# dawn-search/dawnsearch

Measured on AMD Instinct MI355X. Metric: queries/sec, exact cosine top-k over a 384-d f32 index resident in HBM, higher is better.
Workload: dtype f32 (exact scores; int8 MFMA upper-bound filter over 5-bit / int8 shadows)

## Files before the change

### dawnsearch_amd/csrc/scan_f6.hip

```cpp
#include <type_traits>

#include "kernels.hpp"
#include "rotate384.hpp"
#include "wave_topk.hpp"

namespace dawn {

typedef int i32x8_t __attribute__((ext_vector_type(8)));
typedef uint32_t u32x2 __attribute__((ext_vector_type(2)));

constexpr uint32_t F6_KS_DW = 384;
constexpr uint32_t F6_TILE_DW = 3 * F6_KS_DW;
constexpr float F6_MAX = 7.5f;

__device__ __forceinline__ uint32_t f6_encode_mag(float t, float* deq) {
    t = fminf(t, F6_MAX);
    const int e = t < 1.0f ? 0 : t < 2.0f ? 1 : t < 4.0f ? 2 : 3;
    const float step = e <= 1 ? 0.125f : e == 2 ? 0.25f : 0.5f;
    float qn = rintf(t / step);
    if (e == 3) qn = fminf(qn, 15.0f);
    *deq = qn * step;
    const int q = (int)qn;
    return e == 0 ? (uint32_t)q : (uint32_t)((e << 3) + (q - 8));
}
__device__ __forceinline__ uint32_t f6_encode(float v, float inv_s, float* deq) {
    float d;
    const uint32_t c = f6_encode_mag(fabsf(v) * inv_s, &d);
    *deq = v < 0.f ? -d : d;
    return c | (v < 0.f ? 32u : 0u);
}

template <int RT>
__device__ __forceinline__ void rows_to_f6s_pair(const void* __restrict__ xv, uint32_t* __restrict__ out, float2* __restrict__ meta,
                                                 const uint32_t pair, uint32_t n_valid) {
    constexpr int NC = 6;
    __shared__ float sh[4];
    __shared__ float sh_e[4][NC];
    const int tid = threadIdx.x, lane = tid & 63, wave = tid >> 6;
    const uint32_t r = tid >> 3, part = tid & 7;
    const uint32_t row = pair * 32u + r;
    f32x4 v[12];
#pragma unroll
    for (int j = 0; j < 12; ++j) {
        v[j] = f32x4{0.f, 0.f, 0.f, 0.f};
        if (row < n_valid) {
            const uint32_t c4 = part + 8 * j;
            if (RT == 0) {
                v[j] = reinterpret_cast<const f32x4*>(xv)[(size_t)row * ROW_F4 + c4];
            } else {
                const u32x4 w = reinterpret_cast<const u32x4*>(xv)[frag_chunk(row, (int)(c4 >> 1))];
                const uint32_t w0 = (c4 & 1u) ? w.z : w.x, w1 = (c4 & 1u) ? w.w : w.y;
                v[j] = f32x4{bf16_lo(w0), bf16_hi(w0), bf16_lo(w1), bf16_hi(w1)};
            }
        }
    }
    rotate384_rowpart(v, part, lane);
    float amax = 0.f;
#pragma unroll
    for (int j = 0; j < 12; ++j)
        amax = fmaxf(amax, fmaxf(fmaxf(fabsf(v[j].x), fabsf(v[j].y)), fmaxf(fabsf(v[j].z), fabsf(v[j].w))));
#pragma unroll
    for (int o = 32; o >= 1; o >>= 1) amax = fmaxf(amax, __shfl_xor(amax, o));
    if (lane == 0) sh[wave] = amax;
    __syncthreads();
    const int w0 = wave & ~1;
    amax = fmaxf(sh[w0], sh[w0 + 1]);
    const float s0 = fmaxf(amax, 1e-20f) / F6_MAX;
    float e2c[NC];
#pragma unroll
    for (int ci = 0; ci < NC; ++ci) {
        const float inv_s = 1.0f / (s0 * (1.0f - 0.08f * ci)), s = s0 * (1.0f - 0.08f * ci);
        float e2 = 0.f;
#pragma unroll
        for (int j = 0; j < 12; ++j) {
            const float vv[4] = {v[j].x, v[j].y, v[j].z, v[j].w};
#pragma unroll
            for (int i = 0; i < 4; ++i) {
                float dq;
                (void)f6_encode(vv[i], inv_s, &dq);
                const float dx = vv[i] - s * dq;
                e2 = __builtin_fmaf(dx, dx, e2);
            }
        }
        e2 += __shfl_xor(e2, 1);
        e2 += __shfl_xor(e2, 2);
        e2 += __shfl_xor(e2, 4);
#pragma unroll
        for (int o2 = 32; o2 >= 8; o2 >>= 1) e2 = fmaxf(e2, __shfl_xor(e2, o2));
        e2c[ci] = e2;
    }
    if (lane == 0) {
#pragma unroll
        for (int ci = 0; ci < NC; ++ci) sh_e[wave][ci] = e2c[ci];
    }
    __syncthreads();
    float best_e2 = 0.f, s = s0;
#pragma unroll
    for (int ci = 0; ci < NC; ++ci) {
        const float m = fmaxf(sh_e[w0][ci], sh_e[w0 + 1][ci]);
        if (ci == 0 || m < best_e2) {
            best_e2 = m;
            s = s0 * (1.0f - 0.08f * ci);
        }
    }
    const float inv_s = 1.0f / s;
    const uint32_t tile = pair * 2u + (r >> 4), r16 = r & 15u;
    uint32_t* o = out + (size_t)tile * F6_TILE_DW;
    const int base = lane & ~7;
#pragma unroll
    for (int j = 0; j < 12; ++j) {
        const float vv[4] = {v[j].x, v[j].y, v[j].z, v[j].w};
        uint32_t c24 = 0;
#pragma unroll
        for (int i = 0; i < 4; ++i) {
            float dq;
            c24 |= f6_encode(vv[i], inv_s, &dq) << (6 * i);
        }
        const uint32_t c0 = __shfl(c24, base + 0), c1 = __shfl(c24, base + 1), c2 = __shfl(c24, base + 2), c3 = __shfl(c24, base + 3);
        const uint32_t c4 = __shfl(c24, base + 4), c5 = __shfl(c24, base + 5), c6 = __shfl(c24, base + 6), c7 = __shfl(c24, base + 7);
        uint32_t d = 0;
        switch (part) {
            case 0: d = c0 | (c1 << 24); break;
            case 1: d = (c1 >> 8) | (c2 << 16); break;
            case 2: d = (c2 >> 16) | (c3 << 8); break;
            case 3: d = c4 | (c5 << 24); break;
            case 4: d = (c5 >> 8) | (c6 << 16); break;
            case 5: d = (c6 >> 16) | (c7 << 8); break;
            default: break;
        }
        const uint32_t ks = (uint32_t)j >> 2, kb = (uint32_t)j & 3u, l = kb * 16u + r16;
        if (part < 4u) o[ks * F6_KS_DW + l * 4u + part] = d;
        else if (part < 6u) o[ks * F6_KS_DW + 256u + l * 2u + (part - 4u)] = d;
    }
    if ((tid & 127) == 0) {
        meta[tile] = float2{inv_s, sqrtf(best_e2) * 1.0101f * 1.001f + 1e-9f};
    }
}

template <int RT>
__global__ __launch_bounds__(256) void rows_to_f6s_kernel(const void* __restrict__ xv, uint32_t* __restrict__ out,
                                                           float2* __restrict__ meta, uint32_t first_pair, uint32_t n_valid) {
    rows_to_f6s_pair<RT>(xv, out, meta, first_pair + blockIdx.x, n_valid);
}

template <int RT>
__global__ __launch_bounds__(256) void rows_to_f6s_list_kernel(const void* __restrict__ xv, uint32_t* __restrict__ out,
                                                                float2* __restrict__ meta, const uint32_t* __restrict__ list,
                                                                const uint32_t* __restrict__ count, uint32_t end_pair, uint32_t n_valid) {
    if (blockIdx.x >= *count) return;
    const uint32_t pair = list[blockIdx.x];
    if (pair >= end_pair) return;
    rows_to_f6s_pair<RT>(xv, out, meta, pair, n_valid);
}

void launch_rows_to_f6s(const void* d_rows, int rt, void* d_shadow, void* d_meta, size_t first_row, size_t n_valid, hipStream_t stream) {
    const uint32_t first_pair = (uint32_t)(first_row / 32);
    const uint32_t end_pair = (uint32_t)((n_valid + 31) / 32);
    if (end_pair <= first_pair) return;
    if (rt == ROW_BF16)
        hipLaunchKernelGGL(rows_to_f6s_kernel<1>, dim3(end_pair - first_pair), dim3(256), 0, stream, d_rows,
                           reinterpret_cast<uint32_t*>(d_shadow), reinterpret_cast<float2*>(d_meta), first_pair, (uint32_t)n_valid);
    else
        hipLaunchKernelGGL(rows_to_f6s_kernel<0>, dim3(end_pair - first_pair), dim3(256), 0, stream, d_rows,
                           reinterpret_cast<uint32_t*>(d_shadow), reinterpret_cast<float2*>(d_meta), first_pair, (uint32_t)n_valid);
}

void launch_rows_to_f6s_list(const void* d_rows, int rt, void* d_shadow, void* d_meta, const uint32_t* d_list, const uint32_t* d_count,
                             uint32_t max_list, size_t prefix_rows, size_t n_valid, hipStream_t stream) {
    const uint32_t end_pair = (uint32_t)((prefix_rows + 31) / 32);
    if (max_list == 0 || end_pair == 0) return;
    if (rt == ROW_BF16)
        hipLaunchKernelGGL(rows_to_f6s_list_kernel<1>, dim3(max_list), dim3(256), 0, stream, d_rows, reinterpret_cast<uint32_t*>(d_shadow),
                           reinterpret_cast<float2*>(d_meta), d_list, d_count, end_pair, (uint32_t)n_valid);
    else
        hipLaunchKernelGGL(rows_to_f6s_list_kernel<0>, dim3(max_list), dim3(256), 0, stream, d_rows, reinterpret_cast<uint32_t*>(d_shadow),
                           reinterpret_cast<float2*>(d_meta), d_list, d_count, end_pair, (uint32_t)n_valid);
}

__global__ __launch_bounds__(64) void prep_queries_f6_kernel(const float* __restrict__ q, int n_q, uint32_t* __restrict__ qf6,
                                                              float2* __restrict__ qmeta) {
    __shared__ unsigned char codes[EM];
    const int b = blockIdx.x, lane = threadIdx.x;
    float v[6];
#pragma unroll
    for (int j = 0; j < 6; ++j) v[j] = b < n_q ? q[(size_t)b * EM + lane + 64 * j] : 0.f;
    rotate384_wave(v, lane);
    float amax = 0.f;
#pragma unroll
    for (int j = 0; j < 6; ++j) amax = fmaxf(amax, fabsf(v[j]));
#pragma unroll
    for (int o = 32; o >= 1; o >>= 1) amax = fmaxf(amax, __shfl_xor(amax, o));
    const float sq = fmaxf(amax, 1e-20f) / F6_MAX, inv = 1.0f / sq;
    float e2 = 0.f;
#pragma unroll
    for (int j = 0; j < 6; ++j) {
        float dq;
        const uint32_t c = f6_encode(v[j], inv, &dq);
        codes[lane + 64 * j] = b < n_q ? (unsigned char)c : (unsigned char)0;
        const float dx = v[j] - sq * dq;
        e2 = __builtin_fmaf(dx, dx, e2);
    }
#pragma unroll
    for (int o = 32; o >= 1; o >>= 1) e2 += __shfl_xor(e2, o);
    __syncthreads();
    const int g = b >> 4, c16 = b & 15;
    for (int w = lane; w < 72; w += 64) {
        const int kbk = w / 6, d = w % 6;
        uint32_t word = 0;
        const int first = (32 * d) / 6, last = (32 * d + 31) / 6;
        for (int i = first; i <= last && i < 32; ++i) {
            const int sh = 6 * i - 32 * d;
            const uint32_t c = codes[32 * kbk + i];
            word |= sh >= 0 ? (c << sh) : (c >> (-sh));
        }
        const int ks = kbk >> 2, kb = kbk & 3;
        qf6[(((size_t)g * 3 + ks) * 64 + kb * 16 + c16) * 6 + d] = word;
    }
    if (lane == 0) qmeta[b] = float2{sq, b < n_q ? sqrtf(e2) * 1.001f + 1e-9f : 0.f};
}

void launch_prep_queries_f6(const float* d_q, int n_q, void* d_qf6, void* d_qmeta, hipStream_t stream) {
    hipLaunchKernelGGL(prep_queries_f6_kernel, dim3(BATCH_QT), dim3(64), 0, stream, d_q, n_q, reinterpret_cast<uint32_t*>(d_qf6),
                       reinterpret_cast<float2*>(d_qmeta));
}

__device__ __forceinline__ i32x8_t f6_load_a(const uint32_t* tile, int ks, int lane) {
    const u32x4 lo = *reinterpret_cast<const u32x4*>(tile + ks * F6_KS_DW + lane * 4);
    const u32x2 hi = *reinterpret_cast<const u32x2*>(tile + ks * F6_KS_DW + 256 + lane * 2);
    return i32x8_t{(int)lo.x, (int)lo.y, (int)lo.z, (int)lo.w, (int)hi.x, (int)hi.y, 0, 0};
}

__global__ __launch_bounds__(64) void f6_dense_scores_kernel(const uint32_t* __restrict__ x, const float2* __restrict__ meta,
                                                              uint32_t n_rows, const uint32_t* __restrict__ qf6,
                                                              const float2* __restrict__ qmeta, int n_q, float* __restrict__ out) {
    const int lane = threadIdx.x;
    const uint32_t tile = blockIdx.x;
    const uint32_t* t = x + (size_t)tile * F6_TILE_DW;
    const float2 mt = meta[tile];
    const float s = __builtin_amdgcn_rcpf(mt.x);
    i32x8_t a[3];
#pragma unroll
    for (int ks = 0; ks < 3; ++ks) a[ks] = f6_load_a(t, ks, lane);
    for (int g = 0; g * 16 < n_q; ++g) {
        f32x4 acc = {0.f, 0.f, 0.f, 0.f};
#pragma unroll
        for (int ks = 0; ks < 3; ++ks) {
            const uint32_t* bp = qf6 + (((size_t)g * 3 + ks) * 64 + lane) * 6;
            const i32x8_t bv = {(int)bp[0], (int)bp[1], (int)bp[2], (int)bp[3], (int)bp[4], (int)bp[5], 0, 0};
            acc = __builtin_amdgcn_mfma_scale_f32_16x16x128_f8f6f4(a[ks], bv, acc, 2, 2, 0, 0x7F7F7F7F, 0, 0x7F7F7F7F);
        }
        const int qi = 16 * g + (lane & 15);
        const float2 qm = qmeta[qi];
        const float k2 = (1.015f + mt.y) * qm.y;
#pragma unroll
        for (int r = 0; r < 4; ++r) {
            const uint32_t row = tile * 16u + 4u * (uint32_t)(lane >> 4) + (uint32_t)r;
            if (qi < n_q && row < n_rows && row < (uint32_t)BATCH_CAP)
                out[(size_t)qi * BATCH_CAP + row] = __builtin_fmaf(acc[r], s * qm.x, mt.y + k2);
        }
    }
}

void launch_f6_dense_scores(const void* d_f6, const void* d_meta, uint32_t n_rows, const float* d_q, int B, void* d_qf6, void* d_qmeta,
                            float* d_out, hipStream_t stream) {
    launch_prep_queries_f6(d_q, B, d_qf6, d_qmeta, stream);
    const uint32_t n = n_rows < (uint32_t)BATCH_CAP ? n_rows : (uint32_t)BATCH_CAP;
    const uint32_t tiles = (n + 15u) / 16u;
    if (tiles == 0) return;
    hipLaunchKernelGGL(f6_dense_scores_kernel, dim3(tiles), dim3(64), 0, stream, reinterpret_cast<const uint32_t*>(d_f6),
                       reinterpret_cast<const float2*>(d_meta), n_rows, reinterpret_cast<const uint32_t*>(d_qf6),
                       reinterpret_cast<const float2*>(d_qmeta), B, d_out);
}


constexpr int F6_RING = 3;
constexpr uint32_t F6_STAGE = 1344;

template <bool DENSE>
__global__ __launch_bounds__(256) void scan_f6_pass_kernel(const uint32_t* __restrict__ x, const float2* __restrict__ meta, uint32_t n_rows,
                                                            uint32_t stride, uint32_t n_visits, const uint32_t* __restrict__ qf6,
                                                            const float2* __restrict__ qmeta, int n_q, const float* __restrict__ tau,
                                                            uint32_t* __restrict__ cnt, uint2* __restrict__ cand, uint32_t seg_cap,
                                                            float* __restrict__ dense, uint32_t stagger, int mark_lost) {
    __shared__ uint32_t stage[4][F6_STAGE][3];
    const int lane = threadIdx.x & 63;
    const int wave = __builtin_amdgcn_readfirstlane(threadIdx.x >> 6);
    const uint32_t G = gridDim.x;
    const uint32_t n_mine = n_visits > blockIdx.x ? (n_visits - blockIdx.x + G - 1u) / G : 0u;
    const uint32_t p0 = n_mine ? ((uint32_t)wave * stagger) % n_mine : 0u;
    auto visit_of = [&](uint32_t pos) __attribute__((always_inline)) -> uint32_t {
        if (n_mine == 0u) return 0u;
        uint32_t q = p0 + pos;
        q = q >= n_mine ? q - n_mine : q;
        q = q >= n_mine ? q % n_mine : q;
        return blockIdx.x + q * G;
    };
    uint32_t vis = 0;
    u32x4 alo[F6_RING][3];
    u32x2 ahi[F6_RING][3];
#define DAWN_F6_LD4(DST, PTR, OFF) asm volatile("global_load_dwordx4 %0, %1, %2 offset:" #OFF : "=v"(DST) : "v"(off4), "s"(PTR))
#define DAWN_F6_LD2(DST, PTR, OFF) asm volatile("global_load_dwordx2 %0, %1, %2 offset:" #OFF : "=v"(DST) : "v"(off2), "s"(PTR))
    const uint32_t off4 = (uint32_t)lane * 16u, off2 = 1024u + (uint32_t)lane * 8u;
    auto load_tile = [&](int slot, uint32_t v) __attribute__((always_inline)) {
        const uint32_t* p4 = x + (size_t)(v < n_visits ? v * stride : 0u) * F6_TILE_DW;
        const uint32_t* p2 = p4;
        DAWN_F6_LD4(alo[slot][0], p4, 0);
        DAWN_F6_LD2(ahi[slot][0], p2, 0);
        DAWN_F6_LD4(alo[slot][1], p4, 1536);
        DAWN_F6_LD2(ahi[slot][1], p2, 1536);
        DAWN_F6_LD4(alo[slot][2], p4, 3072);
        DAWN_F6_LD2(ahi[slot][2], p2, 3072);
    };
    auto take = [&](int slot, int ks, auto n_tag) __attribute__((always_inline)) -> i32x8_t {
        constexpr int N = decltype(n_tag)::value;
        int o0, o1, o2, o3, o4, o5;
        if constexpr (N >= 0)
            asm volatile("s_waitcnt vmcnt(%12)\n\tv_mov_b32 %0, %6\n\tv_mov_b32 %1, %7\n\tv_mov_b32 %2, %8\n\tv_mov_b32 %3, %9\n\t"
                         "v_mov_b32 %4, %10\n\tv_mov_b32 %5, %11"
                         : "=&v"(o0), "=&v"(o1), "=&v"(o2), "=&v"(o3), "=&v"(o4), "=&v"(o5)
                         : "v"(alo[slot][ks].x), "v"(alo[slot][ks].y), "v"(alo[slot][ks].z), "v"(alo[slot][ks].w), "v"(ahi[slot][ks].x),
                           "v"(ahi[slot][ks].y), "n"(N));
        else
            asm volatile("v_mov_b32 %0, %6\n\tv_mov_b32 %1, %7\n\tv_mov_b32 %2, %8\n\tv_mov_b32 %3, %9\n\tv_mov_b32 %4, %10\n\t"
                         "v_mov_b32 %5, %11"
                         : "=&v"(o0), "=&v"(o1), "=&v"(o2), "=&v"(o3), "=&v"(o4), "=&v"(o5)
                         : "v"(alo[slot][ks].x), "v"(alo[slot][ks].y), "v"(alo[slot][ks].z), "v"(alo[slot][ks].w), "v"(ahi[slot][ks].x),
                           "v"(ahi[slot][ks].y));
        return i32x8_t{o0, o1, o2, o3, o4, o5, 0, 0};
    };
#pragma unroll
    for (int d = 0; d < F6_RING; ++d) load_tile(d, visit_of((uint32_t)d));
    i32x8_t bq[4][3];
    float thrA[4], thrB[4], thrC[4], sq_l[4], dqn_l[4], tau_l[4];
#pragma unroll
    for (int gg = 0; gg < 4; ++gg) {
        const int g = 4 * wave + gg;
        const int qi = 16 * g + (lane & 15);
#pragma unroll
        for (int ks = 0; ks < 3; ++ks) {
            const uint32_t* bp = qf6 + (((size_t)g * 3 + ks) * 64 + lane) * 6;
            const u32x2 b01 = *reinterpret_cast<const u32x2*>(bp), b23 = *reinterpret_cast<const u32x2*>(bp + 2),
                        b45 = *reinterpret_cast<const u32x2*>(bp + 4);
            bq[gg][ks] = i32x8_t{(int)b01.x, (int)b01.y, (int)b23.x, (int)b23.y, (int)b45.x, (int)b45.y, 0, 0};
        }
        const float2 qm = qmeta[qi];
        sq_l[gg] = qm.x;
        dqn_l[gg] = qm.y;
        tau_l[gg] = (!DENSE && qi < n_q) ? tau[qi] : POS_INF;
        thrA[gg] = 1.0f / qm.x;
        thrB[gg] = tau_l[gg] - 1.015f * qm.y;
        thrC[gg] = -(1.0f + qm.y);
    }
    uint32_t n_stage = 0;
    uint32_t(*st)[3] = stage[wave];
    const uint32_t seg = blockIdx.x % (uint32_t)BATCH_CAND_SEGS;
    auto flush = [&]() __attribute__((always_inline)) {
        asm volatile("s_waitcnt lgkmcnt(0)" ::: "memory");
        for (uint32_t i = lane; i < n_stage; i += 64u) {
            const uint32_t ub = st[i][0], row = st[i][1], qi = st[i][2];
            const uint32_t pos = atomicAdd(&cnt[(size_t)qi * BATCH_CAND_SEGS + seg], 1u);
            if (pos < seg_cap) cand[((size_t)qi * BATCH_CAND_SEGS + seg) * seg_cap + pos] = uint2{ub, row};
        }
        n_stage = 0;
    };

    bool lost = false;
    while (vis < n_mine) {
      for (int it = 0; it < 16 && vis < n_mine && (DENSE || n_stage <= F6_STAGE - 1024u); ++it, vis += (uint32_t)F6_RING) {
#pragma unroll
        for (int d = 0; d < F6_RING; ++d) {
            if (vis + (uint32_t)d >= n_mine) break;
            const uint32_t v = visit_of(vis + (uint32_t)d);
            const uint32_t tile = v * stride;
            const float2 mt = meta[tile];
            i32x8_t av[3];
            av[0] = take(d, 0, std::integral_constant<int, 6 * (F6_RING - 1)>());
            av[1] = take(d, 1, std::integral_constant<int, -1>());
            av[2] = take(d, 2, std::integral_constant<int, -1>());
            load_tile(d, visit_of(vis + (uint32_t)d + (uint32_t)F6_RING));
            f32x4 acc[4];
#pragma unroll
            for (int gg = 0; gg < 4; ++gg) {
                acc[gg] = f32x4{0.f, 0.f, 0.f, 0.f};
#pragma unroll
                for (int ks = 0; ks < 3; ++ks)
                    acc[gg] = __builtin_amdgcn_mfma_scale_f32_16x16x128_f8f6f4(av[ks], bq[gg][ks], acc[gg], 2, 2, 0, 0x7F7F7F7F, 0,
                                                                                0x7F7F7F7F);
            }
            const float s = __builtin_amdgcn_rcpf(mt.x);
            const uint32_t row0 = tile * 16u + 4u * (uint32_t)(lane >> 4);
            if constexpr (DENSE) {
#pragma unroll
                for (int gg = 0; gg < 4; ++gg) {
                    const int qi = 16 * (4 * wave + gg) + (lane & 15);
                    const float k2 = (1.015f + mt.y) * dqn_l[gg];
#pragma unroll
                    for (int r = 0; r < 4; ++r) {
                        const uint32_t si = v * 16u + 4u * (uint32_t)(lane >> 4) + (uint32_t)r;
                        if (qi < n_q && si < (uint32_t)BATCH_CAP)
                            dense[(size_t)qi * BATCH_CAP + si] =
                                row0 + (uint32_t)r < n_rows ? __builtin_fmaf(acc[gg][r], s * sq_l[gg], mt.y + k2) : NEG_INF;
                    }
                }
            } else {
                bool any = false;
                float thr[4];
#pragma unroll
                for (int gg = 0; gg < 4; ++gg) {
                    thr[gg] = __builtin_fmaf(__builtin_fmaf(mt.y, thrC[gg], thrB[gg]), mt.x * thrA[gg], -0.02f);
                    any = any || fmaxf(fmaxf(acc[gg][0], acc[gg][1]), fmaxf(acc[gg][2], acc[gg][3])) > thr[gg];
                }
                if (__any(any)) {
#pragma unroll
                    for (int gg = 0; gg < 4; ++gg) {
                        const uint32_t qi = (uint32_t)(16 * (4 * wave + gg) + (lane & 15));
                        const float g1 = s * sq_l[gg], g0 = mt.y + (1.015f + mt.y) * dqn_l[gg];
#pragma unroll
                        for (int r = 0; r < 4; ++r) {
                            const float ub = __builtin_fmaf(acc[gg][r], g1, g0);
                            const bool hit = acc[gg][r] > thr[gg] && ub > tau_l[gg] && row0 + (uint32_t)r < n_rows;
                            const unsigned long long m = __ballot(hit);
                            if (m) {
                                if (hit) {
                                    const uint32_t slot = n_stage + (uint32_t)__popcll(m & ((1ull << lane) - 1ull));
                                    if (slot < F6_STAGE) {
                                        st[slot][0] = __builtin_bit_cast(uint32_t, ub);
                                        st[slot][1] = row0 + (uint32_t)r;
                                        st[slot][2] = qi;
                                    } else {
                                        lost = true;
                                    }
                                }
                                n_stage += (uint32_t)__popcll(m);
                                if (n_stage > F6_STAGE) n_stage = F6_STAGE;
                            }
                        }
                    }
                }
            }
        }
      }
      if (!DENSE && n_stage > 0u) flush();
    }
    asm volatile("s_waitcnt vmcnt(0)" ::: "memory");
#undef DAWN_F6_LD4
#undef DAWN_F6_LD2
    if (!DENSE && mark_lost && __any(lost)) {
        const uint32_t qi = (uint32_t)(64 * wave + lane);
        if ((int)qi < n_q) atomicAdd(&cnt[(size_t)qi * BATCH_CAND_SEGS + seg], seg_cap + 1u);
    }
}

constexpr int F6L_GROUP = 8;
constexpr uint32_t F6L_GROUP_BYTES = F6L_GROUP * F6_TILE_DW * 4u;
constexpr uint32_t F6L_STAGE = 448;
constexpr uint32_t F6L_FLUSH_AT = 192;
struct F6PassLds {
    uint32_t tiles[2][F6L_GROUP_BYTES / 4];
    uint32_t stage[8][F6L_STAGE][3];
};

template <int MODE>
__global__ __launch_bounds__(512) void scan_f6_pass_lds_kernel(const uint32_t* __restrict__ x, const float2* __restrict__ meta,
                                                                uint32_t n_rows, uint32_t n_tiles, const uint32_t* __restrict__ qf6,
                                                                const float2* __restrict__ qmeta, int n_q, const float* __restrict__ tau,
                                                                uint32_t* __restrict__ cnt, uint2* __restrict__ cand, uint32_t seg_cap) {
    extern __shared__ __attribute__((aligned(16))) unsigned char f6l_raw[];
    F6PassLds& L = *reinterpret_cast<F6PassLds*>(f6l_raw);
    const int lane = threadIdx.x & 63;
    const int wave = __builtin_amdgcn_readfirstlane(threadIdx.x >> 6);
    const int qw = wave & 3, half = wave >> 2;
    const uint32_t G = gridDim.x;
    const uint32_t n_groups = (n_tiles + (uint32_t)F6L_GROUP - 1u) / (uint32_t)F6L_GROUP;
    i32x8_t bq[4][3];
    float thrP[4], thrQ[4], sq_l[4], dqn_l[4];
#pragma unroll
    for (int gg = 0; gg < 4; ++gg) {
        const int g = 4 * qw + gg;
        const int qi = 16 * g + (lane & 15);
#pragma unroll
        for (int ks = 0; ks < 3; ++ks) {
            const uint32_t* bp = qf6 + (((size_t)g * 3 + ks) * 64 + lane) * 6;
            const u32x2 b01 = *reinterpret_cast<const u32x2*>(bp), b23 = *reinterpret_cast<const u32x2*>(bp + 2),
                        b45 = *reinterpret_cast<const u32x2*>(bp + 4);
            bq[gg][ks] = i32x8_t{(int)b01.x, (int)b01.y, (int)b23.x, (int)b23.y, (int)b45.x, (int)b45.y, 0, 0};
        }
        const float2 qm = qmeta[qi];
        sq_l[gg] = qm.x;
        dqn_l[gg] = qm.y;
        const float tau_q = qi < n_q ? tau[qi] : POS_INF;
        thrP[gg] = (tau_q - 1.015f * qm.y) / qm.x;
        thrQ[gg] = -(1.0f + qm.y) / qm.x;
    }
    uint32_t n_stage = 0;
    uint32_t(*st)[3] = L.stage[wave];
    const uint32_t seg = blockIdx.x % (uint32_t)BATCH_CAND_SEGS;
    bool lost = false;

    const uint32_t lds0 = (uint32_t)(size_t)(__attribute__((address_space(3))) unsigned char*)f6l_raw;
    const uint32_t o4 = (uint32_t)threadIdx.x * 16u, o2 = 32768u + (uint32_t)threadIdx.x * 8u, om = (uint32_t)(lane & 7) * 8u;
    const uint32_t o4b = o4 + 8192u, o4c = o4 + 16384u, o4d = o4 + 24576u;
    u32x4 pa0, pa1, pa2, pa3, pb0, pb1, pb2, pb3;
    u32x2 pa4, pb4, pam, pbm;
#define DAWN_F6L_PREFETCH(P0, P1, P2, P3, P4, PM, GRP)                                                                         \
    do {                                                                                                                      \
        const uint32_t g_ = (GRP) < n_groups ? (GRP) : n_groups - 1u;         \
        const unsigned char* xb_ = reinterpret_cast<const unsigned char*>(x) + (size_t)g_ * F6L_GROUP_BYTES;                  \
        const float2* mb_ = meta + (size_t)g_ * F6L_GROUP;                                                                    \
        asm volatile("global_load_dwordx4 %0, %6, %11 nt\n\tglobal_load_dwordx4 %1, %7, %11 nt\n\t"                           \
                     "global_load_dwordx4 %2, %8, %11 nt\n\tglobal_load_dwordx4 %3, %9, %11 nt\n\t"                           \
                     "global_load_dwordx2 %4, %10, %11 nt\n\tglobal_load_dwordx2 %5, %12, %13"                                \
                     : "=&v"(P0), "=&v"(P1), "=&v"(P2), "=&v"(P3), "=&v"(P4), "=&v"(PM)                                       \
                     : "v"(o4), "v"(o4b), "v"(o4c), "v"(o4d), "v"(o2), "s"(xb_), "v"(om), "s"(mb_)                            \
                     : "memory");                                                                                             \
    } while (0)
#define DAWN_F6L_LAND(P0, P1, P2, P3, P4, PM, BUF, MX, MY)                                                                     \
    do {                                                                                                                      \
        const uint32_t a4_ = lds0 + (BUF) + o4, a2_ = lds0 + (BUF) + (uint32_t)threadIdx.x * 8u;                              \
        asm volatile("s_waitcnt vmcnt(6)\n\tds_write_b128 %2, %4\n\tds_write_b128 %2, %5 offset:8192\n\t"                    \
                     "ds_write_b128 %2, %6 offset:16384\n\tds_write_b128 %2, %7 offset:24576\n\t"                            \
                     "ds_write_b64 %3, %8 offset:32768\n\tv_mov_b32 %0, %9\n\tv_mov_b32 %1, %10"                             \
                     : "=&v"(MX), "=&v"(MY)                                                                                   \
                     : "v"(a4_), "v"(a2_), "v"(P0), "v"(P1), "v"(P2), "v"(P3), "v"(P4), "v"(PM.x), "v"(PM.y)                  \
                     : "memory");                                                                                             \
    } while (0)
#define DAWN_F6L_BARRIER() asm volatile("s_waitcnt lgkmcnt(0)\n\ts_barrier" ::: "memory")

    auto compute = [&](const unsigned char* tb, uint32_t grp, int cmx, int cmy, auto mid) __attribute__((always_inline)) {
        auto read_tile = [&](int t, i32x8_t (&av)[3]) __attribute__((always_inline)) {
#pragma unroll
            for (int ks = 0; ks < 3; ++ks) {
                const unsigned char* f = tb + (uint32_t)t * (F6_TILE_DW * 4u) + (uint32_t)ks * (F6_KS_DW * 4u);
                const u32x4 lo = *reinterpret_cast<const u32x4*>(f + lane * 16);
                const u32x2 hi = *reinterpret_cast<const u32x2*>(f + 1024 + lane * 8);
                av[ks] = i32x8_t{(int)lo.x, (int)lo.y, (int)lo.z, (int)lo.w, (int)hi.x, (int)hi.y, 0, 0};
            }
        };
        constexpr int NT = F6L_GROUP / 2;
        i32x8_t av[2][3];
        f32x4 acc[2][4];
        read_tile(half, av[0]);
#pragma unroll
        for (int k = 0; k <= NT; ++k) {
            if (k + 1 < NT) read_tile(half + 2 * (k + 1), av[(k + 1) & 1]);
            if (k < NT) {
#pragma unroll
                for (int gg = 0; gg < 4; ++gg) acc[k & 1][gg] = f32x4{0.f, 0.f, 0.f, 0.f};
#pragma unroll
                for (int ks = 0; ks < 3; ++ks)
#pragma unroll
                    for (int gg = 0; gg < 4; ++gg)
                        acc[k & 1][gg] = __builtin_amdgcn_mfma_scale_f32_16x16x128_f8f6f4(av[k & 1][ks], bq[gg][ks], acc[k & 1][gg], 2, 2, 0,
                                                                                           0x7F7F7F7F, 0, 0x7F7F7F7F);
            }
            if (k >= 1) {
                const int t = half + 2 * (k - 1);
                const f32x4(&ac)[4] = acc[(k - 1) & 1];
                const uint32_t tile = grp * (uint32_t)F6L_GROUP + (uint32_t)t;
                const float2 mt = float2{__builtin_bit_cast(float, __builtin_amdgcn_readlane(cmx, t)),
                                         __builtin_bit_cast(float, __builtin_amdgcn_readlane(cmy, t))};
                const float sx = mt.x, sxy = mt.x * mt.y;
                unsigned long long mk[4][4], any_m = 0ull;
                float thr[4];
#pragma unroll
                for (int gg = 0; gg < 4; ++gg) {
                    thr[gg] = __builtin_fmaf(sx, thrP[gg], __builtin_fmaf(sxy, thrQ[gg], -0.02f));
#pragma unroll
                    for (int r = 0; r < 4; ++r) {
                        mk[gg][r] = __ballot(ac[gg][r] > thr[gg]);
                        any_m |= mk[gg][r];
                    }
                }
                if (MODE != 1 && any_m != 0ull) {
                    const float s = __builtin_amdgcn_rcpf(mt.x);
                    const uint32_t row0 = tile * 16u + 4u * (uint32_t)(lane >> 4);
#pragma unroll
                    for (int gg = 0; gg < 4; ++gg) {
                        if ((mk[gg][0] | mk[gg][1] | mk[gg][2] | mk[gg][3]) == 0ull) continue;
                        const uint32_t qi = (uint32_t)(16 * (4 * qw + gg) + (lane & 15));
                        const float g1 = s * sq_l[gg], g0 = mt.y + (1.015f + mt.y) * dqn_l[gg];
#pragma unroll
                        for (int r = 0; r < 4; ++r) {
                            if (mk[gg][r] == 0ull) continue;
                            const bool hit = ac[gg][r] > thr[gg] && row0 + (uint32_t)r < n_rows;
                            const unsigned long long m = __ballot(hit);
                            if (hit) {
                                const uint32_t slot = n_stage + (uint32_t)__popcll(m & ((1ull << lane) - 1ull));
                                if (slot < F6L_STAGE) {
                                    st[slot][0] = __builtin_bit_cast(uint32_t, __builtin_fmaf(ac[gg][r], g1, g0));
                                    st[slot][1] = row0 + (uint32_t)r;
                                    st[slot][2] = qi;
                                } else {
                                    lost = true;
                                }
                            }
                            n_stage += (uint32_t)__popcll(m);
                            if (n_stage > F6L_STAGE) n_stage = F6L_STAGE;
                        }
                    }
                }
                if constexpr (MODE == 1) {
                    const float sum = (ac[0][0] + ac[1][1]) + (ac[2][2] + ac[3][3]);
                    if (sum == 1.2345e30f) lost = true;
                }
            }
            if (k == 1) mid();
        }
    };
    auto flush = [&]() __attribute__((always_inline)) {
        for (uint32_t i = lane; i < n_stage; i += 64u) {
            const uint32_t ub = st[i][0], row = st[i][1], qi = st[i][2];
            const uint32_t pos = atomicAdd(&cnt[(size_t)qi * BATCH_CAND_SEGS + seg], 1u);
            if (pos < seg_cap) cand[((size_t)qi * BATCH_CAND_SEGS + seg) * seg_cap + pos] = uint2{ub, row};
        }
        n_stage = 0;
        asm volatile("s_waitcnt vmcnt(0)" ::: "memory");
    };

    uint32_t grp = blockIdx.x;
    if (grp < n_groups) {
        const unsigned char* tb0 = reinterpret_cast<const unsigned char*>(L.tiles[0]);
        const unsigned char* tb1 = reinterpret_cast<const unsigned char*>(L.tiles[1]);
        int mx0, my0, mx1, my1;
        DAWN_F6L_PREFETCH(pa0, pa1, pa2, pa3, pa4, pam, grp);
        DAWN_F6L_PREFETCH(pb0, pb1, pb2, pb3, pb4, pbm, grp + G);
        DAWN_F6L_LAND(pa0, pa1, pa2, pa3, pa4, pam, 0u, mx0, my0);
        DAWN_F6L_PREFETCH(pa0, pa1, pa2, pa3, pa4, pam, grp + 2u * G);
        DAWN_F6L_BARRIER();
        unsigned long long t_land = 0, t_bar = 0, t_all = 0, t0 = 0, n_it = 0;
#define DAWN_F6L_T() (MODE == 4 ? __builtin_readcyclecounter() : 0ull)
        t_all = DAWN_F6L_T();
        while (true) {
            compute(tb0, grp, mx0, my0, [&]() __attribute__((always_inline)) {
                t0 = DAWN_F6L_T();
                DAWN_F6L_LAND(pb0, pb1, pb2, pb3, pb4, pbm, F6L_GROUP_BYTES, mx1, my1);
                t_land += DAWN_F6L_T() - t0;
                DAWN_F6L_PREFETCH(pb0, pb1, pb2, pb3, pb4, pbm, grp + 3u * G);
            });
            t0 = DAWN_F6L_T();
            DAWN_F6L_BARRIER();
            t_bar += DAWN_F6L_T() - t0;
            ++n_it;
            grp += G;
            if (grp >= n_groups) break;
            compute(tb1, grp, mx1, my1, [&]() __attribute__((always_inline)) {
                t0 = DAWN_F6L_T();
                DAWN_F6L_LAND(pa0, pa1, pa2, pa3, pa4, pam, 0u, mx0, my0);
                t_land += DAWN_F6L_T() - t0;
                DAWN_F6L_PREFETCH(pa0, pa1, pa2, pa3, pa4, pam, grp + 3u * G);
            });
            t0 = DAWN_F6L_T();
            DAWN_F6L_BARRIER();
            t_bar += DAWN_F6L_T() - t0;
            ++n_it;
            grp += G;
            if (grp >= n_groups) break;
            if (n_stage > F6L_FLUSH_AT) flush();
        }
        asm volatile("s_waitcnt vmcnt(0)" ::: "memory");
        if constexpr (MODE == 4) {
            t_all = DAWN_F6L_T() - t_all;
            if (lane == 0 && (blockIdx.x == 0 || blockIdx.x == 131) && (wave == 0 || wave == 5))
                printf("f6 pass timing: block %d wave %d: %llu groups, shader cycles total %llu, landing %llu, barrier %llu\n",
                       (int)blockIdx.x, wave, n_it, t_all, t_land, t_bar);
        }
#undef DAWN_F6L_T
        if (n_stage > 0u) flush();
    }
#undef DAWN_F6L_PREFETCH
#undef DAWN_F6L_LAND
#undef DAWN_F6L_BARRIER
    if (__any(lost)) {
        const uint32_t qi = (uint32_t)(64 * qw + lane);
        if ((int)qi < n_q) atomicAdd(&cnt[(size_t)qi * BATCH_CAND_SEGS + seg], seg_cap + 1u);
    }
}



__global__ __launch_bounds__(256) void f6_refine_kernel(const uint2* __restrict__ big, uint32_t* __restrict__ cnt_big, uint32_t seg_cap_big,
                                                         const unsigned char* __restrict__ x8, const float2* __restrict__ meta8,
                                                         const signed char* __restrict__ qi8, const float2* __restrict__ qm8,
                                                         float* __restrict__ tau, uint32_t* __restrict__ cnt, uint2* __restrict__ cand) {
    __shared__ __attribute__((aligned(16))) signed char sh_img[EM];
    __shared__ uint32_t sh_cnt;
    const int b = blockIdx.x, seg = blockIdx.y;
    for (int i = threadIdx.x; i < EM / 4; i += blockDim.x)
        reinterpret_cast<int*>(sh_img)[i] = reinterpret_cast<const int*>(qi8 + (size_t)b * EM)[i];
    if (threadIdx.x == 0) {
        const uint32_t c = cnt_big[(size_t)b * BATCH_CAND_SEGS + seg];
        sh_cnt = c <= seg_cap_big ? c : 0u;
    }
    __syncthreads();
    const uint32_t n = sh_cnt;
    const float2 qm = qm8[b];
    const float t = tau[b];
    const uint2* src = big + ((size_t)b * BATCH_CAND_SEGS + seg) * seg_cap_big;
    const i32x4_t* img = reinterpret_cast<const i32x4_t*>(sh_img);
    for (uint32_t e = threadIdx.x; e < n; e += blockDim.x) {
        const uint2 v = src[e];
        const float ub6 = __builtin_bit_cast(float, v.x);
        const uint32_t row = v.y;
        const uint32_t t8 = row >> 5, r8 = row & 31u;
        const i32x4_t* xs = reinterpret_cast<const i32x4_t*>(x8 + (size_t)t8 * 12288u) + r8;
        int c = 0;
#pragma unroll 6
        for (int j = 0; j < 24; ++j) {
            const i32x4_t xv = xs[(j >> 1) * 64 + (j & 1) * 32];
            const i32x4_t hv = img[j];
            c = __builtin_amdgcn_sdot4(xv[0], hv[0], c, false);
            c = __builtin_amdgcn_sdot4(xv[1], hv[1], c, false);
            c = __builtin_amdgcn_sdot4(xv[2], hv[2], c, false);
            c = __builtin_amdgcn_sdot4(xv[3], hv[3], c, false);
        }
        const float2 m8 = meta8[t8];
        const float ub8 = __builtin_fmaf((float)c, __builtin_amdgcn_rcpf(m8.x) * qm.x, m8.y + qm.y);
        const float ub = fminf(ub6, ub8);
        if (ub > t) {
            const uint32_t pos = atomicAdd(&cnt[(size_t)b * BATCH_CAND_SEGS + seg], 1u);
            if (pos < (uint32_t)BATCH_CAP / (uint32_t)BATCH_CAND_SEGS)
                cand[((size_t)b * BATCH_CAND_SEGS + seg) * ((uint32_t)BATCH_CAP / (uint32_t)BATCH_CAND_SEGS) + pos] =
                    uint2{__builtin_bit_cast(uint32_t, ub), row};
        }
    }
    __syncthreads();
    if (threadIdx.x == 0) {
        if (cnt_big[(size_t)b * BATCH_CAND_SEGS + seg] > seg_cap_big) tau[b] = POS_INF;
        cnt_big[(size_t)b * BATCH_CAND_SEGS + seg] = 0u;
    }
}

__global__ __launch_bounds__(256) void f6_refine_rows_kernel(const uint2* __restrict__ big, uint32_t* __restrict__ cnt_big,
                                                              uint32_t seg_cap_big, const f32x4* __restrict__ x,
                                                              const float* __restrict__ q, float* __restrict__ tau,
                                                              uint32_t* __restrict__ cnt, uint2* __restrict__ cand) {
    const int b = blockIdx.x, seg = blockIdx.y;
    const int part = threadIdx.x & 15, grp = threadIdx.x >> 4;
    f32x4 qv[6];
#pragma unroll
    for (int j = 0; j < 6; ++j) qv[j] = reinterpret_cast<const f32x4*>(q + (size_t)b * EM)[part + 16 * j];
    const uint32_t c0 = cnt_big[(size_t)b * BATCH_CAND_SEGS + seg];
    const uint32_t n = c0 <= seg_cap_big ? c0 : 0u;
    const float t = tau[b];
    const uint2* src = big + ((size_t)b * BATCH_CAND_SEGS + seg) * seg_cap_big;
    constexpr uint32_t seg_small = (uint32_t)BATCH_CAP / (uint32_t)BATCH_CAND_SEGS;
    for (uint32_t e0 = 0; e0 < n; e0 += 32u) {
        const uint32_t ea = e0 + (uint32_t)grp, eb = ea + 16u;
        const uint2 va = ea < n ? src[ea] : uint2{0u, 0u}, vb = eb < n ? src[eb] : uint2{0u, 0u};
        const f32x4* ra = x + (size_t)va.y * ROW_F4 + part;
        const f32x4* rb = x + (size_t)vb.y * ROW_F4 + part;
        f32x4 xa[6], xb[6];
#pragma unroll
        for (int j = 0; j < 6; ++j) {
            xa[j] = __builtin_nontemporal_load(ra + 16 * j);
            xb[j] = __builtin_nontemporal_load(rb + 16 * j);
        }
        float da = 0.f, db = 0.f;
#pragma unroll
        for (int j = 0; j < 6; ++j) {
            da = __builtin_fmaf(xa[j].x, qv[j].x, da);
            da = __builtin_fmaf(xa[j].y, qv[j].y, da);
            da = __builtin_fmaf(xa[j].z, qv[j].z, da);
            da = __builtin_fmaf(xa[j].w, qv[j].w, da);
            db = __builtin_fmaf(xb[j].x, qv[j].x, db);
            db = __builtin_fmaf(xb[j].y, qv[j].y, db);
            db = __builtin_fmaf(xb[j].z, qv[j].z, db);
            db = __builtin_fmaf(xb[j].w, qv[j].w, db);
        }
#pragma unroll
        for (int o = 8; o >= 1; o >>= 1) {
            da += __shfl_xor(da, o);
            db += __shfl_xor(db, o);
        }
        if (part == 0) {
#pragma unroll
            for (int h = 0; h < 2; ++h) {
                const uint32_t e = h ? eb : ea;
                const uint2 v = h ? vb : va;
                const float ub = fminf(__builtin_bit_cast(float, v.x), (h ? db : da) + 3e-5f);
                if (e < n && ub > t) {
                    const uint32_t pos = atomicAdd(&cnt[(size_t)b * BATCH_CAND_SEGS + seg], 1u);
                    if (pos < seg_small) cand[((size_t)b * BATCH_CAND_SEGS + seg) * seg_small + pos] = uint2{__builtin_bit_cast(uint32_t, ub), v.y};
                }
            }
        }
    }
    __syncthreads();
    if (threadIdx.x == 0) {
        if (c0 > seg_cap_big) tau[b] = POS_INF;
        cnt_big[(size_t)b * BATCH_CAND_SEGS + seg] = 0u;
    }
}

__global__ void f6_merge_tau_kernel(float* __restrict__ tau, float* __restrict__ tau6, int n, int have_tau8) {
    const int i = threadIdx.x;
    if (i < n) {
        const float t = have_tau8 ? fmaxf(tau[i], tau6[i]) : tau6[i];
        tau[i] = t;
        tau6[i] = t;
    }
}

struct F6Plan {
    uint32_t n_tiles, s1_tiles, s1_stride, m1, s2_tiles, s2_stride, m2;
};
static F6Plan plan_f6(uint32_t n_rows, uint32_t target) {
    F6Plan pl{};
    pl.n_tiles = (n_rows + 15u) / 16u;
    pl.s1_tiles = (uint32_t)BATCH_CAP / 16u;
    if (pl.s1_tiles > pl.n_tiles) pl.s1_tiles = pl.n_tiles;
    pl.s1_stride = pl.n_tiles / pl.s1_tiles;
    uint32_t t2 = pl.n_tiles / 64u;
    if (t2 > 1500000u / 16u) t2 = 1500000u / 16u;
    if (t2 < 1024u) t2 = 1024u;
    if (t2 > pl.n_tiles) t2 = pl.n_tiles;
    pl.s2_tiles = t2;
    pl.s2_stride = pl.n_tiles / t2;
    const double n2 = (double)t2 * 16.0;
    double m2 = (double)target * n2 / (double)n_rows;
    if (m2 < 16.0) m2 = 16.0;
    if (m2 > 2048.0) m2 = 2048.0;
    pl.m2 = (uint32_t)(m2 + 0.5);
    double m1 = 4.0 * m2 * (double)(pl.s1_tiles * 16u) / n2;
    if (m1 < 4.0) m1 = 4.0;
    if (m1 > 256.0) m1 = 256.0;
    pl.m1 = (uint32_t)(m1 + 0.999);
    return pl;
}

void launch_scan_batched_f6(const void* d_x, int dtype, const void* d_i8, const void* d_i8meta, const void* d_f6, const void* d_f6meta,
                            const uint64_t* d_ids, uint32_t n_rows, const float* d_q, int B, uint32_t k, const BatchWorkspace& ws,
                            const F6Workspace& f6, int grid, uint64_t* d_labels, float* d_dist, uint32_t* d_found, uint32_t* d_flags,
                            int force_fallback, hipStream_t stream, hipEvent_t ev0, hipEvent_t ev1) {
    const bool rows_refine = dtype == ROW_F32 && f6.refine_rows;
    if (!rows_refine) launch_i8_sample_thresholds(d_i8, d_i8meta, n_rows, d_q, B, k, ws, grid, stream);
    const uint32_t target = (uint32_t)f6.target * (k > 32 ? 2u : 1u);
    const F6Plan pl = plan_f6(n_rows, target);
    const uint32_t* xs = reinterpret_cast<const uint32_t*>(d_f6);
    const float2* mt = reinterpret_cast<const float2*>(d_f6meta);
    const uint32_t* qf6 = reinterpret_cast<const uint32_t*>(f6.qf6);
    const float2* qm6 = reinterpret_cast<const float2*>(f6.qmeta);
    launch_prep_queries_f6(d_q, B, f6.qf6, f6.qmeta, stream);
    BatchWorkspace w6 = ws;
    w6.tau = f6.tau6;
    const uint32_t seg_small = (uint32_t)BATCH_CAP / (uint32_t)BATCH_CAND_SEGS;
    {
        const uint32_t blocks = pl.s1_tiles < (uint32_t)grid ? pl.s1_tiles : (uint32_t)grid;
        hipLaunchKernelGGL(scan_f6_pass_kernel<true>, dim3(blocks), dim3(256), 0, stream, xs, mt, n_rows, pl.s1_stride, pl.s1_tiles, qf6,
                           qm6, B, f6.tau6, ws.cnt, reinterpret_cast<uint2*>(ws.cand), seg_small, reinterpret_cast<float*>(ws.cand), 0u, 0);
        launch_tau_select(true, B, w6, pl.s1_tiles * 16u, pl.m1, stream);
    }
    {
        const uint32_t blocks = pl.s2_tiles < 2u * (uint32_t)grid ? pl.s2_tiles : 2u * (uint32_t)grid;
        hipLaunchKernelGGL(scan_f6_pass_kernel<false>, dim3(blocks), dim3(256), 0, stream, xs, mt, n_rows, pl.s2_stride, pl.s2_tiles, qf6,
                           qm6, B, f6.tau6, ws.cnt, reinterpret_cast<uint2*>(ws.cand), seg_small, reinterpret_cast<float*>(ws.cand), 0u, 0);
        launch_tau_select(false, B, w6, 0u, pl.m2, stream);
    }
    hipLaunchKernelGGL(f6_merge_tau_kernel, dim3(1), dim3(256), 0, stream, ws.tau, f6.tau6, B, rows_refine ? 0 : 1);
    if (ev0) (void)hipEventRecord(ev0, stream);
    if (f6.stagger < 0) {
        static OncePerDevice attr_once;
        once_per_device(attr_once, [] {
            (void)hipFuncSetAttribute(reinterpret_cast<const void*>(scan_f6_pass_lds_kernel<0>), hipFuncAttributeMaxDynamicSharedMemorySize,
                                      (int)sizeof(F6PassLds));
#ifdef DAWN_EXPERIMENTS
            (void)hipFuncSetAttribute(reinterpret_cast<const void*>(scan_f6_pass_lds_kernel<1>), hipFuncAttributeMaxDynamicSharedMemorySize,
                                      (int)sizeof(F6PassLds));
            (void)hipFuncSetAttribute(reinterpret_cast<const void*>(scan_f6_pass_lds_kernel<4>), hipFuncAttributeMaxDynamicSharedMemorySize,
                                      (int)sizeof(F6PassLds));
#endif
        });
        const uint32_t n_groups = (pl.n_tiles + (uint32_t)F6L_GROUP - 1u) / (uint32_t)F6L_GROUP;
        const uint32_t blocks = n_groups < (uint32_t)grid ? n_groups : (uint32_t)grid;
#ifdef DAWN_EXPERIMENTS
        auto kern = f6.stagger == -2 ? scan_f6_pass_lds_kernel<1> : f6.stagger == -4 ? scan_f6_pass_lds_kernel<4> : scan_f6_pass_lds_kernel<0>;
#else
        auto kern = scan_f6_pass_lds_kernel<0>;
#endif
        hipLaunchKernelGGL(kern, dim3(blocks), dim3(512), sizeof(F6PassLds), stream, xs, mt, n_rows, pl.n_tiles, qf6, qm6, B, f6.tau6,
                           f6.cnt_big, reinterpret_cast<uint2*>(f6.cand_big), f6.seg_cap_big);
    } else {
        const uint32_t blocks = pl.n_tiles < (uint32_t)grid ? pl.n_tiles : (uint32_t)grid;
        hipLaunchKernelGGL(scan_f6_pass_kernel<false>, dim3(blocks), dim3(256), 0, stream, xs, mt, n_rows, 1u, pl.n_tiles, qf6, qm6, B,
                           f6.tau6, f6.cnt_big, reinterpret_cast<uint2*>(f6.cand_big), f6.seg_cap_big, nullptr, (uint32_t)f6.stagger, 1);
    }
    if (ev1) (void)hipEventRecord(ev1, stream);
    const signed char* qi8 = reinterpret_cast<const signed char*>(ws.qh);
    const float2* qm8 = reinterpret_cast<const float2*>(qi8 + (size_t)BATCH_QT * EM);
    if (rows_refine)
        hipLaunchKernelGGL(f6_refine_rows_kernel, dim3(B, BATCH_CAND_SEGS), dim3(256), 0, stream,
                           reinterpret_cast<const uint2*>(f6.cand_big), f6.cnt_big, f6.seg_cap_big, reinterpret_cast<const f32x4*>(d_x),
                           d_q, ws.tau, ws.cnt, reinterpret_cast<uint2*>(ws.cand));
    else
        hipLaunchKernelGGL(f6_refine_kernel, dim3(B, BATCH_CAND_SEGS), dim3(256), 0, stream, reinterpret_cast<const uint2*>(f6.cand_big),
                           f6.cnt_big, f6.seg_cap_big, reinterpret_cast<const unsigned char*>(d_i8),
                           reinterpret_cast<const float2*>(d_i8meta), qi8, qm8, ws.tau, ws.cnt, reinterpret_cast<uint2*>(ws.cand));
    launch_select_rescore_eps(false, d_x, dtype, d_ids, n_rows, d_q, B, k, ws, d_labels, d_dist, d_found, d_flags, force_fallback,
                              FILTER_EPS_I8, stream);
}

}
```

Baseline: 290.4.

## Run stage-2 sample pass on LDS-pipelined scan kernel and streamline candidate staging

The strided stage-2 threshold sampling pass now runs on the LDS double-buffered 512-thread kernel instead of the older per-tile scan kernel. Sampling switches from tiles to 8-tile groups with a group stride. The hit test in the hot loop first reduces each accumulator to a per-query max with a single ballot, and only computes per-row ballots for groups with a hit. Staged candidates are written with exec-masked inline LDS stores whose slots come from mbcnt, and a padding row is added to the stage array. The intent is to cut ballot and branch overhead in the filter and to speed up the sampling pass, at the cost of a different sample set (contiguous groups) and more hand-written assembly.

```diff
diff --git a/dawnsearch_amd/csrc/scan_f6.hip b/dawnsearch_amd/csrc/scan_f6.hip
--- a/dawnsearch_amd/csrc/scan_f6.hip
+++ b/dawnsearch_amd/csrc/scan_f6.hip
@@ -1,3 +1,4 @@
+#include <cstddef>
 #include <type_traits>
 
 #include "kernels.hpp"
@@ -457,21 +458,24 @@
 constexpr uint32_t F6L_FLUSH_AT = 192;
 struct F6PassLds {
     uint32_t tiles[2][F6L_GROUP_BYTES / 4];
-    uint32_t stage[8][F6L_STAGE][3];
+    uint32_t stage[8][F6L_STAGE + 1][3];
 };
+__device__ __forceinline__ float f6_max4(float a, float b, float c, float d) {
+    return __builtin_elementwise_maximum(__builtin_elementwise_maximum(a, b), __builtin_elementwise_maximum(c, d));
+}
 
 template <int MODE>
 __global__ __launch_bounds__(512) void scan_f6_pass_lds_kernel(const uint32_t* __restrict__ x, const float2* __restrict__ meta,
-                                                                uint32_t n_rows, uint32_t n_tiles, const uint32_t* __restrict__ qf6,
-                                                                const float2* __restrict__ qmeta, int n_q, const float* __restrict__ tau,
-                                                                uint32_t* __restrict__ cnt, uint2* __restrict__ cand, uint32_t seg_cap) {
+                                                                uint32_t n_rows, uint32_t n_groups, uint32_t gstride,
+                                                                const uint32_t* __restrict__ qf6, const float2* __restrict__ qmeta, int n_q,
+                                                                const float* __restrict__ tau, uint32_t* __restrict__ cnt,
+                                                                uint2* __restrict__ cand, uint32_t seg_cap, int mark_lost) {
     extern __shared__ __attribute__((aligned(16))) unsigned char f6l_raw[];
     F6PassLds& L = *reinterpret_cast<F6PassLds*>(f6l_raw);
     const int lane = threadIdx.x & 63;
     const int wave = __builtin_amdgcn_readfirstlane(threadIdx.x >> 6);
     const int qw = wave & 3, half = wave >> 2;
     const uint32_t G = gridDim.x;
-    const uint32_t n_groups = (n_tiles + (uint32_t)F6L_GROUP - 1u) / (uint32_t)F6L_GROUP;
     i32x8_t bq[4][3];
     float thrP[4], thrQ[4], sq_l[4], dqn_l[4];
 #pragma unroll
@@ -500,11 +504,12 @@
     const uint32_t lds0 = (uint32_t)(size_t)(__attribute__((address_space(3))) unsigned char*)f6l_raw;
     const uint32_t o4 = (uint32_t)threadIdx.x * 16u, o2 = 32768u + (uint32_t)threadIdx.x * 8u, om = (uint32_t)(lane & 7) * 8u;
     const uint32_t o4b = o4 + 8192u, o4c = o4 + 16384u, o4d = o4 + 24576u;
+    const uint32_t st_lds = lds0 + (uint32_t)offsetof(F6PassLds, stage) + (uint32_t)wave * (F6L_STAGE + 1u) * 12u;
     u32x4 pa0, pa1, pa2, pa3, pb0, pb1, pb2, pb3;
     u32x2 pa4, pb4, pam, pbm;
 #define DAWN_F6L_PREFETCH(P0, P1, P2, P3, P4, PM, GRP)                                                                         \
     do {                                                                                                                      \
-        const uint32_t g_ = (GRP) < n_groups ? (GRP) : n_groups - 1u;         \
+        const uint32_t g_ = ((GRP) < n_groups ? (GRP) : n_groups - 1u) * gstride;  \
         const unsigned char* xb_ = reinterpret_cast<const unsigned char*>(x) + (size_t)g_ * F6L_GROUP_BYTES;                  \
         const float2* mb_ = meta + (size_t)g_ * F6L_GROUP;                                                                    \
         asm volatile("global_load_dwordx4 %0, %6, %11 nt\n\tglobal_load_dwordx4 %1, %7, %11 nt\n\t"                           \
@@ -556,47 +561,58 @@
             if (k >= 1) {
                 const int t = half + 2 * (k - 1);
                 const f32x4(&ac)[4] = acc[(k - 1) & 1];
-                const uint32_t tile = grp * (uint32_t)F6L_GROUP + (uint32_t)t;
+                const uint32_t tile = grp * gstride * (uint32_t)F6L_GROUP + (uint32_t)t;
                 const float2 mt = float2{__builtin_bit_cast(float, __builtin_amdgcn_readlane(cmx, t)),
                                          __builtin_bit_cast(float, __builtin_amdgcn_readlane(cmy, t))};
                 const float sx = mt.x, sxy = mt.x * mt.y;
-                unsigned long long mk[4][4], any_m = 0ull;
-                float thr[4];
+                float thr[4], mx[4];
 #pragma unroll
                 for (int gg = 0; gg < 4; ++gg) {
                     thr[gg] = __builtin_fmaf(sx, thrP[gg], __builtin_fmaf(sxy, thrQ[gg], -0.02f));
-#pragma unroll
-                    for (int r = 0; r < 4; ++r) {
-                        mk[gg][r] = __ballot(ac[gg][r] > thr[gg]);
-                        any_m |= mk[gg][r];
-                    }
+                    mx[gg] = f6_max4(ac[gg][0], ac[gg][1], ac[gg][2], ac[gg][3]);
                 }
-                if (MODE != 1 && any_m != 0ull) {
+                const float d = f6_max4(mx[0] - thr[0], mx[1] - thr[1], mx[2] - thr[2], mx[3] - thr[3]);
+                if (MODE != 1 && __ballot(d >= 0.f) != 0ull) {
                     const float s = __builtin_amdgcn_rcpf(mt.x);
                     const uint32_t row0 = tile * 16u + 4u * (uint32_t)(lane >> 4);
+                    const int rem = (int)(n_rows - (uint32_t)__builtin_amdgcn_readfirstlane(tile) * 16u);
 #pragma unroll
                     for (int gg = 0; gg < 4; ++gg) {
-                        if ((mk[gg][0] | mk[gg][1] | mk[gg][2] | mk[gg][3]) == 0ull) continue;
+                        if (__ballot(mx[gg] > thr[gg]) == 0ull) continue;
+                        unsigned long long m[4];
+#pragma unroll
+                        for (int r = 0; r < 4; ++r) m[r] = __ballot(ac[gg][r] > thr[gg]);
+                        if (rem < 16) {
+#pragma unroll
+                            for (int r = 0; r < 4; ++r) {
+                                const int nb = rem > r ? (rem - r + 3) >> 2 : 0;
+                                if (nb < 4) m[r] &= (1ull << (16 * nb)) - 1ull;
+                            }
+                        }
+                        const uint32_t c0 = (uint32_t)__popcll(m[0]), c1 = (uint32_t)__popcll(m[1]), c2 = (uint32_t)__popcll(m[2]);
+                        const uint32_t c3 = (uint32_t)__popcll(m[3]);
+                        const uint32_t base[4] = {n_stage, n_stage + c0, n_stage + c0 + c1, n_stage + c0 + c1 + c2};
+                        const uint32_t n_new = base[3] + c3;
                         const uint32_t qi = (uint32_t)(16 * (4 * qw + gg) + (lane & 15));
                         const float g1 = s * sq_l[gg], g0 = mt.y + (1.015f + mt.y) * dqn_l[gg];
 #pragma unroll
                         for (int r = 0; r < 4; ++r) {
-                            if (mk[gg][r] == 0ull) continue;
-                            const bool hit = ac[gg][r] > thr[gg] && row0 + (uint32_t)r < n_rows;
-                            const unsigned long long m = __ballot(hit);
-                            if (hit) {
-                                const uint32_t slot = n_stage + (uint32_t)__popcll(m & ((1ull << lane) - 1ull));
-                                if (slot < F6L_STAGE) {
-                                    st[slot][0] = __builtin_bit_cast(uint32_t, __builtin_fmaf(ac[gg][r], g1, g0));
-                                    st[slot][1] = row0 + (uint32_t)r;
-                                    st[slot][2] = qi;
-                                } else {
-                                    lost = true;
-                                }
-                            }
-                            n_stage += (uint32_t)__popcll(m);
-                            if (n_stage > F6L_STAGE) n_stage = F6L_STAGE;
+                            if (m[r] == 0ull) continue;
+                            uint32_t slot = __builtin_amdgcn_mbcnt_hi((uint32_t)(m[r] >> 32),
+                                                                      __builtin_amdgcn_mbcnt_lo((uint32_t)m[r], base[r]));
+                            slot = slot < F6L_STAGE ? slot : F6L_STAGE;
+                            const uint32_t a = st_lds + slot * 12u;
+                            const float ub = __builtin_fmaf(ac[gg][r], g1, g0);
+                            const uint32_t row = row0 + (uint32_t)r;
+                            unsigned long long sv;
+                            asm volatile("s_mov_b64 %0, exec\n\ts_mov_b64 exec, %1\n\tds_write2_b32 %2, %3, %4 offset1:1\n\t"
+                                         "ds_write_b32 %2, %5 offset:8\n\ts_mov_b64 exec, %0"
+                                         : "=&s"(sv)
+                                         : "s"(m[r]), "v"(a), "v"(ub), "v"(row), "v"(qi)
+                                         : "memory");
                         }
+                        if (n_new > F6L_STAGE) lost = true;
+                        n_stage = n_new < F6L_STAGE ? n_new : F6L_STAGE;
                     }
                 }
                 if constexpr (MODE == 1) {
@@ -670,7 +686,7 @@
 #undef DAWN_F6L_PREFETCH
 #undef DAWN_F6L_LAND
 #undef DAWN_F6L_BARRIER
-    if (__any(lost)) {
+    if (mark_lost && lost) {
         const uint32_t qi = (uint32_t)(64 * qw + lane);
         if ((int)qi < n_q) atomicAdd(&cnt[(size_t)qi * BATCH_CAND_SEGS + seg], seg_cap + 1u);
     }
@@ -802,21 +818,24 @@
 }
 
 struct F6Plan {
-    uint32_t n_tiles, s1_tiles, s1_stride, m1, s2_tiles, s2_stride, m2;
+    uint32_t n_tiles, n_groups, s1_tiles, s1_stride, m1, s2_groups, s2_gstride, m2;
 };
 static F6Plan plan_f6(uint32_t n_rows, uint32_t target) {
     F6Plan pl{};
     pl.n_tiles = (n_rows + 15u) / 16u;
+    pl.n_groups = (pl.n_tiles + (uint32_t)F6L_GROUP - 1u) / (uint32_t)F6L_GROUP;
     pl.s1_tiles = (uint32_t)BATCH_CAP / 16u;
     if (pl.s1_tiles > pl.n_tiles) pl.s1_tiles = pl.n_tiles;
     pl.s1_stride = pl.n_tiles / pl.s1_tiles;
     uint32_t t2 = pl.n_tiles / 64u;
     if (t2 > 1500000u / 16u) t2 = 1500000u / 16u;
     if (t2 < 1024u) t2 = 1024u;
-    if (t2 > pl.n_tiles) t2 = pl.n_tiles;
-    pl.s2_tiles = t2;
-    pl.s2_stride = pl.n_tiles / t2;
-    const double n2 = (double)t2 * 16.0;
+    uint32_t g2 = (t2 + (uint32_t)F6L_GROUP - 1u) / (uint32_t)F6L_GROUP;
+    if (g2 > pl.n_groups) g2 = pl.n_groups;
+    pl.s2_groups = g2;
+    pl.s2_gstride = pl.n_groups / g2;
+    double n2 = (double)g2 * (16.0 * F6L_GROUP);
+    if (n2 > (double)n_rows) n2 = (double)n_rows;
     double m2 = (double)target * n2 / (double)n_rows;
     if (m2 < 16.0) m2 = 16.0;
     if (m2 > 2048.0) m2 = 2048.0;
@@ -850,35 +869,34 @@
                            qm6, B, f6.tau6, ws.cnt, reinterpret_cast<uint2*>(ws.cand), seg_small, reinterpret_cast<float*>(ws.cand), 0u, 0);
         launch_tau_select(true, B, w6, pl.s1_tiles * 16u, pl.m1, stream);
     }
+    static OncePerDevice attr_once;
+    once_per_device(attr_once, [] {
+        (void)hipFuncSetAttribute(reinterpret_cast<const void*>(scan_f6_pass_lds_kernel<0>), hipFuncAttributeMaxDynamicSharedMemorySize,
+                                  (int)sizeof(F6PassLds));
+#ifdef DAWN_EXPERIMENTS
+        (void)hipFuncSetAttribute(reinterpret_cast<const void*>(scan_f6_pass_lds_kernel<1>), hipFuncAttributeMaxDynamicSharedMemorySize,
+                                  (int)sizeof(F6PassLds));
+        (void)hipFuncSetAttribute(reinterpret_cast<const void*>(scan_f6_pass_lds_kernel<4>), hipFuncAttributeMaxDynamicSharedMemorySize,
+                                  (int)sizeof(F6PassLds));
+#endif
+    });
     {
-        const uint32_t blocks = pl.s2_tiles < 2u * (uint32_t)grid ? pl.s2_tiles : 2u * (uint32_t)grid;
-        hipLaunchKernelGGL(scan_f6_pass_kernel<false>, dim3(blocks), dim3(256), 0, stream, xs, mt, n_rows, pl.s2_stride, pl.s2_tiles, qf6,
-                           qm6, B, f6.tau6, ws.cnt, reinterpret_cast<uint2*>(ws.cand), seg_small, reinterpret_cast<float*>(ws.cand), 0u, 0);
+        const uint32_t blocks = pl.s2_groups < (uint32_t)grid ? pl.s2_groups : (uint32_t)grid;
+        hipLaunchKernelGGL(scan_f6_pass_lds_kernel<0>, dim3(blocks), dim3(512), sizeof(F6PassLds), stream, xs, mt, n_rows, pl.s2_groups,
+                           pl.s2_gstride, qf6, qm6, B, f6.tau6, ws.cnt, reinterpret_cast<uint2*>(ws.cand), seg_small, 0);
         launch_tau_select(false, B, w6, 0u, pl.m2, stream);
     }
     hipLaunchKernelGGL(f6_merge_tau_kernel, dim3(1), dim3(256), 0, stream, ws.tau, f6.tau6, B, rows_refine ? 0 : 1);
     if (ev0) (void)hipEventRecord(ev0, stream);
     if (f6.stagger < 0) {
-        static OncePerDevice attr_once;
-        once_per_device(attr_once, [] {
-            (void)hipFuncSetAttribute(reinterpret_cast<const void*>(scan_f6_pass_lds_kernel<0>), hipFuncAttributeMaxDynamicSharedMemorySize,
-                                      (int)sizeof(F6PassLds));
-#ifdef DAWN_EXPERIMENTS
-            (void)hipFuncSetAttribute(reinterpret_cast<const void*>(scan_f6_pass_lds_kernel<1>), hipFuncAttributeMaxDynamicSharedMemorySize,
-                                      (int)sizeof(F6PassLds));
-            (void)hipFuncSetAttribute(reinterpret_cast<const void*>(scan_f6_pass_lds_kernel<4>), hipFuncAttributeMaxDynamicSharedMemorySize,
-                                      (int)sizeof(F6PassLds));
-#endif
-        });
-        const uint32_t n_groups = (pl.n_tiles + (uint32_t)F6L_GROUP - 1u) / (uint32_t)F6L_GROUP;
-        const uint32_t blocks = n_groups < (uint32_t)grid ? n_groups : (uint32_t)grid;
+        const uint32_t blocks = pl.n_groups < (uint32_t)grid ? pl.n_groups : (uint32_t)grid;
 #ifdef DAWN_EXPERIMENTS
         auto kern = f6.stagger == -2 ? scan_f6_pass_lds_kernel<1> : f6.stagger == -4 ? scan_f6_pass_lds_kernel<4> : scan_f6_pass_lds_kernel<0>;
 #else
         auto kern = scan_f6_pass_lds_kernel<0>;
 #endif
-        hipLaunchKernelGGL(kern, dim3(blocks), dim3(512), sizeof(F6PassLds), stream, xs, mt, n_rows, pl.n_tiles, qf6, qm6, B, f6.tau6,
-                           f6.cnt_big, reinterpret_cast<uint2*>(f6.cand_big), f6.seg_cap_big);
+        hipLaunchKernelGGL(kern, dim3(blocks), dim3(512), sizeof(F6PassLds), stream, xs, mt, n_rows, pl.n_groups, 1u, qf6, qm6, B, f6.tau6,
+                           f6.cnt_big, reinterpret_cast<uint2*>(f6.cand_big), f6.seg_cap_big, 1);
     } else {
         const uint32_t blocks = pl.n_tiles < (uint32_t)grid ? pl.n_tiles : (uint32_t)grid;
         hipLaunchKernelGGL(scan_f6_pass_kernel<false>, dim3(blocks), dim3(256), 0, stream, xs, mt, n_rows, 1u, pl.n_tiles, qf6, qm6, B,
```

Result: no change. 290.3, median of 6 (-0.0%).
